# Sylphy0052/Othello_Reinforcement_learning_test

Hardware: AMD Instinct MI355X
Metric: self-play games/sec (8x8, 50 MCTS sims/move) (higher is better)
Workload: dtype f16x3 (fp16 hi/lo operand split on MFMA, fp32 accumulate; fp32-equivalent)

## Files before the change

othello_reinforcement_learning_test_amd/csrc/net_wino.hip:

```cpp
#include <math.h>
#include <stdlib.h>
#include <string.h>

#include <type_traits>
#include <vector>

#include "net.h"
#include "net_heads.h"
#include "net_epilogue.h"

namespace oth {

using half8 = _Float16 __attribute__((ext_vector_type(8)));
using half4 = _Float16 __attribute__((ext_vector_type(4)));
using f32x4 = float __attribute__((ext_vector_type(4)));

constexpr int kWTile = 512;
constexpr int kWVBytes = 2 * 32 * 4 * kWTile;
constexpr int kWZeroOff = kWVBytes;
constexpr int kWLds = kWVBytes + 4 * kWTile;
constexpr float kWClamp = 30000.0f;

struct WinoWeights {
    int blocks = 0;
    uint4* d_w = nullptr;
    uint4* d_stem = nullptr;
    float* d_bias = nullptr;
    float* d_inv = nullptr;
    float* d_pfc_wt = nullptr;
    float* d_vfc1_wt = nullptr;
};

struct WinoArgs {
    const uint4* w;
    const uint4* stem;
    const float* bias;
    const float* inv;
    int n_res_layers;
    HeadParams heads;
    const float* pfc_wt;
    const float* vfc1_wt;
    int* sat;
    float act_scale;
    unsigned long long* dbg;
};

#ifdef OTH_STAMPS
__device__ __forceinline__ unsigned long long w_clk() {
    unsigned long long t;
    __builtin_amdgcn_sched_barrier(0);
    asm volatile("s_memtime %0\n\ts_waitcnt lgkmcnt(0)" : "=s"(t)::"memory");
    __builtin_amdgcn_sched_barrier(0);
    return t;
}
__device__ __forceinline__ unsigned long long w_realclk() {
    unsigned long long t;
    __builtin_amdgcn_sched_barrier(0);
    asm volatile("s_memrealtime %0\n\ts_waitcnt lgkmcnt(0)" : "=s"(t)::"memory");
    __builtin_amdgcn_sched_barrier(0);
    return t;
}
#define OTH_WSTAMP(i) { const unsigned long long t1_ = w_clk(); ph_[i] += t1_ - t0_; t0_ = t1_; }
#else
#define OTH_WSTAMP(i)
#endif

__device__ __forceinline__ f32x4 wmfma(half8 a, half8 b, f32x4 c) {
    asm volatile("v_mfma_f32_16x16x32_f16 %0, %1, %2, %0" : "+v"(c) : "v"(a), "v"(b));
    return c;
}
__device__ __forceinline__ f32x4 wmfma0(half8 a, half8 b) {
    f32x4 c;
    asm volatile("v_mfma_f32_16x16x32_f16 %0, %1, %2, 0" : "=v"(c) : "v"(a), "v"(b));
    return c;
}
__device__ __forceinline__ void wbarrier() {
    asm volatile("s_waitcnt lgkmcnt(0)" ::: "memory");
    __builtin_amdgcn_s_barrier();
    asm volatile("" ::: "memory");
}
__device__ __forceinline__ float quad_prev(float v) {
    return __builtin_bit_cast(float, __builtin_amdgcn_mov_dpp(__builtin_bit_cast(int, v), 0x90, 0xf, 0xf, true));
}
__device__ __forceinline__ float quad_next(float v) {
    return __builtin_bit_cast(float, __builtin_amdgcn_mov_dpp(__builtin_bit_cast(int, v), 0xF9, 0xf, 0xf, true));
}

#define OTH_WSB __builtin_amdgcn_sched_barrier(0)
constexpr int kHeadRow = 129;

__device__ __forceinline__ void heads_block2(const HeadParams& hp, const float* __restrict__ pfc_wt,
                                             const float* __restrict__ vfc1_wt, const float* act, float* scratch,
                                             bool live1, float* __restrict__ logp, float* __restrict__ vout,
                                             unsigned long long* hst = nullptr) {
    const int t = threadIdx.x;
#ifdef OTH_STAMPS
    unsigned long long h0_ = w_clk();
#define OTH_HST(i) { const unsigned long long h1_ = w_clk(); if (hst) hst[i] = h1_ - h0_; h0_ = h1_; }
#else
#define OTH_HST(i)
#endif
    float* w3 = scratch;
    float* feat = scratch + 384;
    float* h1 = scratch + 768;
    float* lgp = scratch + 1280;
    if (t < 384) {
        const int i = t / 3, k = t % 3;
        w3[t] = k < 2 ? hp.pconv_w[i * 2 + k] : hp.vconv_w[i];
    }
    __syncthreads();
    if (t < 384) {
        const int p = t / 192, rem = t % 192, k = rem >> 6, cell = rem & 63;
        const float* a = act + (size_t)(p * 64 + cell) * kHeadRow;
        float p0 = 0.f, p1 = 0.f;
#pragma unroll 16
        for (int i = 0; i < 128; i += 2) {
            p0 = fmaf(a[i], w3[i * 3 + k], p0);
            p1 = fmaf(a[i + 1], w3[(i + 1) * 3 + k], p1);
        }
        float acc = p0 + p1;
        acc += k < 2 ? hp.pconv_b[k] : hp.vconv_b[0];
        feat[p * 192 + k * 64 + cell] = acc > 0.f ? acc : 0.f;
    }
    __syncthreads();
    OTH_HST(0)
    if (t < 256) {
        float a0 = hp.vfc1_b[t], a1 = a0;
#pragma unroll
        for (int i = 0; i < 64; ++i) {
            const float w = vfc1_wt[i * 256 + t];
            a0 = fmaf(w, feat[128 + i], a0);
            a1 = fmaf(w, feat[192 + 128 + i], a1);
        }
        h1[t] = a0 > 0.f ? a0 : 0.f;
        h1[256 + t] = a1 > 0.f ? a1 : 0.f;
    } else if (t < 256 + 130) {
        const int u = t - 256, o = u % 65, part = u / 65;
        float s0 = part == 0 ? hp.pfc_b[o] : 0.f, s1 = s0;
#pragma unroll
        for (int i = 0; i < 64; ++i) {
            const float w = pfc_wt[(part * 64 + i) * 65 + o];
            s0 = fmaf(w, feat[part * 64 + i], s0);
            s1 = fmaf(w, feat[192 + part * 64 + i], s1);
        }
        lgp[part * 72 + o] = s0;
        lgp[(2 + part) * 72 + o] = s1;
    }
    OTH_HST(1)
    __syncthreads();
    if ((t & 255) < 64) {
        const int p = t >> 8, l = t & 63;
        const float* gp = lgp + p * 2 * 72;
        const float gl = gp[l] + gp[72 + l];
        const float g64 = gp[64] + gp[72 + 64];
        float m = fmaxf(gl, l == 0 ? g64 : -INFINITY);
        m = bfly_max_f32(m);
        float s = expf(gl - m) + (l == 0 ? expf(g64 - m) : 0.f);
        s = bfly_sum_f32(s);
        const float lse = logf(s);
        float acc = 0.f;
        for (int i = l; i < 256; i += 64) acc = fmaf(hp.vfc2_w[i], h1[p * 256 + i], acc);
        acc = bfly_sum_f32(acc);
        if (p == 0 || live1) {
            logp[p * 65 + l] = gl - m - lse;
            if (l == 0) {
                logp[p * 65 + 64] = g64 - m - lse;
                vout[p] = tanhf(acc + hp.vfc2_b[0]);
            }
        }
    }
}

template <int TP>
__global__ __launch_bounds__(512, 2) void k_trunk_w(WinoArgs a, const uint64_t* __restrict__ sb,
                                                    const uint64_t* __restrict__ ob, const uint64_t* __restrict__ lgl,
                                                    int64_t n, const int32_t* __restrict__ n_valid,
                                                    float* __restrict__ logp, float* __restrict__ vout) {
    extern __shared__ __attribute__((aligned(16))) char lds[];
#ifdef OTH_STAMPS
    const unsigned long long tentry_ = w_clk();
#endif
    int64_t nv = n;
    if (n_valid) {
        const int64_t k = *n_valid;
        nv = k < n ? k : n;
    }
    constexpr int NT = 2 * TP;
    const int64_t pos0 = (int64_t)blockIdx.x * TP;
    if (pos0 >= nv) return;
    const int tid = threadIdx.x, lane = tid & 63, wave = tid >> 6;
    const int g4 = lane >> 4, c = lane & 15;
    const int row4 = c >> 2, j = c & 3;

    if (tid < TP * 64) {
        const int p = tid >> 6, cell = tid & 63, y = cell >> 3, x = cell & 7;
        const bool live = pos0 + p < nv;
        const uint64_t b0 = live ? sb[pos0 + p] : 0, b1 = live ? ob[pos0 + p] : 0, b2 = live ? lgl[pos0 + p] : 0;
        const _Float16 one = (x & 1) ? (_Float16)(-a.act_scale) : (_Float16)a.act_scale;
        _Float16 vals[32];
#pragma unroll
        for (int i = 0; i < 32; ++i) vals[i] = (_Float16)0.0f;
#pragma unroll
        for (int tap = 0; tap < 9; ++tap) {
            const int yy = y + tap / 3 - 1, xx = x + tap % 3 - 1;
            const bool ok = yy >= 0 && yy < 8 && xx >= 0 && xx < 8;
            const int s = ok ? yy * 8 + xx : 0;
            vals[tap * 3 + 0] = (ok && ((b0 >> s) & 1ULL)) ? one : (_Float16)0.0f;
            vals[tap * 3 + 1] = (ok && ((b1 >> s) & 1ULL)) ? one : (_Float16)0.0f;
            vals[tap * 3 + 2] = (ok && ((b2 >> s) & 1ULL)) ? one : (_Float16)0.0f;
        }
        half8* dst = (half8*)(lds + tid * 64);
#pragma unroll
        for (int q = 0; q < 4; ++q) {
            half8 t;
#pragma unroll
            for (int i = 0; i < 8; ++i) t[i] = vals[q * 8 + i];
            dst[q] = t;
        }
    }
    if (tid < 128) ((uint4*)(lds + kWZeroOff))[tid] = make_uint4(0, 0, 0, 0);
    __syncthreads();

    f32x4 acc[4][NT];
    f32x4 res[NT][2];
#pragma unroll
    for (int xi = 0; xi < 4; ++xi)
#pragma unroll
        for (int nt = 0; nt < NT; ++nt) {
            acc[xi][nt] = f32x4{0.f, 0.f, 0.f, 0.f};
            OTH_PIN_ACC(acc[xi][nt]);
        }
    OTH_PIN_ACC_END();
#pragma unroll
    for (int nt = 0; nt < NT; ++nt) res[nt][0] = res[nt][1] = f32x4{0.f, 0.f, 0.f, 0.f};

    {
        const uint4* wp = a.stem + (size_t)wave * 2 * 64 + lane;
        const half8 wh = __builtin_bit_cast(half8, wp[0]), wlo = __builtin_bit_cast(half8, wp[64]);
#pragma unroll
        for (int nt = 0; nt < NT; ++nt)
#pragma unroll
            for (int e = 0; e < 2; ++e) {
                const int cell = (nt >> 1) * 64 + ((nt & 1) * 4 + row4) * 8 + 2 * j + e;
                const half8 xh = *(const half8*)(lds + cell * 64 + g4 * 16);
                acc[3 * e][nt] = wmfma(wlo, xh, acc[3 * e][nt]);
                acc[3 * e][nt] = wmfma(wh, xh, acc[3 * e][nt]);
            }
    }

    const int ch0 = wave * 16 + 4 * g4;
    const uint32_t wchunk = (uint32_t)(2 * wave + (g4 >> 1));
    uint32_t wr_off[NT];
#pragma unroll
    for (int nt = 0; nt < NT; ++nt) {
        const uint32_t tl = (uint32_t)((nt & 1) * 16 + c);
        wr_off[nt] = ((uint32_t)(nt >> 1) * 32 + tl) * (4 * kWTile) + ((wchunk ^ (tl & 15)) << 4) + 8u * (uint32_t)(g4 & 1);
    }
    uint32_t rd_base[NT][3];
    uint32_t rd_key[3];
#pragma unroll
    for (int d = 0; d < 3; ++d) {
        rd_key[d] = ((uint32_t)((c + 4 * (d - 1)) & 15) << 4) ^ ((uint32_t)g4 << 4);
#pragma unroll
        for (int nt = 0; nt < NT; ++nt) {
            const int y = (nt & 1) * 4 + row4 + (d - 1);
            const int ts = (nt & 1) * 16 + c + 4 * (d - 1);
            rd_base[nt][d] = (y >= 0 && y < 8) ? (uint32_t)((nt >> 1) * 32 + ts) * (4 * kWTile) : (uint32_t)kWZeroOff;
        }
    }
    const float mask_l = j == 0 ? 0.f : 1.f, mask_r = j == 3 ? 0.f : 1.f;
    const f32x2 mask_l2 = {mask_l, mask_l}, mask_r2 = {mask_r, mask_r};

    const int n_layers = 1 + a.n_res_layers;
    uint32_t sat_bits = 0;
    constexpr int RING = TP == 1 ? 4 : 2;
    static_assert(12 % RING == 0, "the ring index must be a compile-time function of the group");
    uint4 wq[RING][8];
#ifdef OTH_STAMPS
    unsigned long long ph_[4] = {0, 0, 0, 0}, t0_ = w_clk(), tstart_ = t0_;
    const unsigned long long rstart_ = w_realclk();
#endif
    float4 b4 = *(const float4*)(a.bias + ch0), b4n = b4;
    float inv = a.inv[0], invn = inv;
    for (int layer = 0; layer < n_layers; ++layer) {
        const bool last = layer == n_layers - 1;
        if (layer > 0) {
            b4 = b4n;
            inv = invn;
        }
        const f32x2 inv2 = {inv, inv};
        const uint4* wl = a.w + (size_t)layer * (12 * 8 * 8 * 64) + (size_t)wave * (8 * 64) + lane;
        auto epilogue = [&](auto SKIP) {
            constexpr bool add_res = decltype(SKIP)::value;
#pragma unroll
            for (int nt = 0; nt < NT; ++nt) {
                f32x2 v0[2], v1[2];
#pragma unroll
                for (int h = 0; h < 2; ++h) {
                    const f32x2 a0 = whalf(acc[0][nt], h), a1 = whalf(acc[1][nt], h), a2 = whalf(acc[2][nt], h),
                                a3 = whalf(acc[3][nt], h);
                    const f32x2 bb = h == 0 ? f32x2{b4.x, b4.y} : f32x2{b4.z, b4.w};
                    const f32x2 t0 = pk_fma(pk_add(pk_add(a0, a1), a2), inv2, bb);
                    const f32x2 t1 = pk_fma(pk_sub(pk_sub(a1, a2), a3), inv2, bb);
                    if (add_res) {
                        f32x2 r0 = whalf(res[nt][0], h), r1 = whalf(res[nt][1], h);
                        pk_add_relu_inplace(r0, t0, kWClamp);
                        pk_add_relu_inplace(r1, t1, kWClamp);
                        wsethalf(res[nt][0], h, r0);
                        wsethalf(res[nt][1], h, r1);
                        v0[h] = r0;
                        v1[h] = r1;
                    } else {
                        v0[h] = f32x2{__builtin_amdgcn_fmed3f(t0.x, 0.f, kWClamp), __builtin_amdgcn_fmed3f(t0.y, 0.f, kWClamp)};
                        v1[h] = f32x2{__builtin_amdgcn_fmed3f(t1.x, 0.f, kWClamp), __builtin_amdgcn_fmed3f(t1.y, 0.f, kWClamp)};
                    }
                }
                sat_bits = max(sat_bits, max(max(__float_as_uint(v0[0].x), __float_as_uint(v0[0].y)),
                                             max(__float_as_uint(v0[1].x), __float_as_uint(v0[1].y))));
                sat_bits = max(sat_bits, max(max(__float_as_uint(v1[0].x), __float_as_uint(v1[0].y)),
                                             max(__float_as_uint(v1[1].x), __float_as_uint(v1[1].y))));
                if (!last) {
                    f32x2 V[4][2];
#pragma unroll
                    for (int h = 0; h < 2; ++h) {
                        const f32x2 dl = {quad_prev(v1[h].x), quad_prev(v1[h].y)};
                        const f32x2 dr = {quad_next(v0[h].x), quad_next(v0[h].y)};
                        V[0][h] = pk_fma_nc(dl, mask_l2, v1[h]);
                        V[1][h] = pk_add(v0[h], v1[h]);
                        V[2][h] = pk_sub(v1[h], v0[h]);
                        V[3][h] = pk_fma_na(dr, mask_r2, v0[h]);
                    }
#pragma unroll
                    for (int xi = 0; xi < 4; ++xi) {
                        uint2 hi, lo;
                        hi.x = wpack(V[xi][0].x, V[xi][0].y);
                        hi.y = wpack(V[xi][1].x, V[xi][1].y);
                        lo.x = wresid(hi.x, V[xi][0].x, V[xi][0].y);
                        lo.y = wresid(hi.y, V[xi][1].x, V[xi][1].y);
                        char* dst = lds + wr_off[nt] + xi * kWTile;
                        *(uint2*)dst = hi;
                        *(uint2*)(dst + 256) = lo;
                    }
                }
                OTH_WSB;
            }
        };
        using T_ = std::true_type;
        using F_ = std::false_type;
        if (layer == 0 && !last) {
#pragma unroll
            for (int g = 0; g < RING - 1; ++g)
#pragma unroll
                for (int f = 0; f < 8; ++f) wq[g][f] = wl[(size_t)g * (8 * 8 * 64) + (size_t)f * 64];
        }
        OTH_WSTAMP(0)
        wbarrier();
        OTH_WSTAMP(1)
        if (layer & 1) epilogue(F_{});
        else epilogue(T_{});
        if (last) break;
        OTH_WSTAMP(2)
        wbarrier();
        OTH_WSTAMP(1)

        constexpr int GS = NT * 4;
        constexpr int QT = 12 * GS;
        auto src_of = [&](int q) -> const char* {
            const int xi = q & 3, nt = (q >> 2) % NT, grp = q / GS, kk = grp & 3, d = grp >> 2;
            return lds + rd_base[nt][d] + ((uint32_t)(kk << 6) ^ rd_key[d]) + xi * kWTile;
        };
        constexpr int PD = 2;
        half8 xh[PD + 1], xl[PD + 1];
#pragma unroll
        for (int q = 0; q < PD; ++q) {
            xh[q] = *(const half8*)src_of(q);
            xl[q] = *(const half8*)(src_of(q) + 256);
        }
        auto conv_d = [&](auto DC) {
            constexpr int D = decltype(DC)::value;
#pragma unroll
            for (int ql = 0; ql < 4 * GS; ++ql) {
                const int q = D * 4 * GS + ql;
                const int xi = q & 3, nt = (q >> 2) % NT, grp = q / GS, sl = q % (PD + 1), psl = (q + PD) % (PD + 1);
                const int step = q % GS;
                const half8 wh = __builtin_bit_cast(half8, wq[grp % RING][2 * xi]);
                const half8 wlo = __builtin_bit_cast(half8, wq[grp % RING][2 * xi + 1]);
                OTH_WSB;
                if (q < GS) acc[xi][nt] = wmfma0(wh, xl[sl]);
                else acc[xi][nt] = wmfma(wh, xl[sl], acc[xi][nt]);
                OTH_WSB;
                if (q + PD < QT) xh[psl] = *(const half8*)src_of(q + PD);
                OTH_WSB;
                acc[xi][nt] = wmfma(wh, xh[sl], acc[xi][nt]);
                OTH_WSB;
                if (q + PD < QT) xl[psl] = *(const half8*)(src_of(q + PD) + 256);
                if (grp == 10 && step == GS / 2) {
                    b4n = *(const float4*)(a.bias + (layer + 1) * 128 + ch0);
                    invn = a.inv[layer + 1];
                }
                if (step < 8)
                    wq[(grp + RING - 1) % RING][step] = wl[(size_t)(grp + RING - 1) * (8 * 8 * 64) + (size_t)step * 64];
                OTH_WSB;
                acc[xi][nt] = wmfma(wlo, xh[sl], acc[xi][nt]);
                OTH_WSB;
            }
        };
        conv_d(std::integral_constant<int, 0>{});
        conv_d(std::integral_constant<int, 1>{});
        conv_d(std::integral_constant<int, 2>{});
        OTH_WSTAMP(3)
    }
#ifdef OTH_STAMPS
    if (a.dbg && lane == 0) {
        unsigned long long* o = a.dbg + ((size_t)blockIdx.x * 8 + wave) * 8;
        for (int i = 0; i < 4; ++i) o[i] = ph_[i];
        o[4] = w_clk() - tstart_;
        o[5] = w_realclk() - rstart_;
        o[6] = rstart_;
        o[7] = tstart_ - tentry_;
    }
    const unsigned long long theads_ = w_clk();
#endif

    if (sat_bits >= __float_as_uint(kWClamp)) atomicOr(a.sat, 1);
    __syncthreads();
#pragma unroll
    for (int nt = 0; nt < NT; ++nt)
#pragma unroll
        for (int e = 0; e < 2; ++e) {
            const int cell = (nt >> 1) * 64 + ((nt & 1) * 4 + row4) * 8 + 2 * j + e;
            const float us = 1.0f / a.act_scale;
            const f32x4 v = res[nt][e];
            float* dst = (float*)lds + (size_t)cell * kHeadRow + ch0;
            dst[0] = v[0] * us;
            dst[1] = v[1] * us;
            dst[2] = v[2] * us;
            dst[3] = v[3] * us;
        }
    __syncthreads();
#ifdef OTH_STAMPS
    unsigned long long hst_[2] = {0, 0};
    const unsigned long long tpre_ = w_clk() - theads_;
    heads_block2(a.heads, a.pfc_wt, a.vfc1_wt, (const float*)lds, (float*)(lds + 128 * kHeadRow * 4 + 64), TP == 2 && pos0 + 1 < nv,
                 logp + pos0 * 65, vout + pos0, hst_);
#if OTH_STAMPS != 2
    if (a.dbg && lane == 0) {
        unsigned long long* o = a.dbg + ((size_t)blockIdx.x * 8 + wave) * 8;
        o[3] = w_clk() - theads_;
        o[0] = tpre_; o[1] = hst_[0]; o[2] = hst_[1];
    }
#endif
#else
    heads_block2(a.heads, a.pfc_wt, a.vfc1_wt, (const float*)lds, (float*)(lds + 128 * kHeadRow * 4 + 64), TP == 2 && pos0 + 1 < nv,
                 logp + pos0 * 65, vout + pos0);
#endif
}

static inline void wsplit(float v, uint16_t& hi, uint16_t& lo) {
    const _Float16 hh = (_Float16)v;
    const _Float16 ll = (_Float16)(v - (float)hh);
    memcpy(&hi, &hh, 2);
    memcpy(&lo, &ll, 2);
}

void wino_free_weights(oth_net* net) {
    if (!net->wino) return;
    WinoWeights* w = net->wino;
    if (w->d_w) (void)hipFree(w->d_w);
    if (w->d_stem) (void)hipFree(w->d_stem);
    if (w->d_bias) (void)hipFree(w->d_bias);
    if (w->d_inv) (void)hipFree(w->d_inv);
    if (w->d_pfc_wt) (void)hipFree(w->d_pfc_wt);
    if (w->d_vfc1_wt) (void)hipFree(w->d_vfc1_wt);
    delete w;
    net->wino = nullptr;
}

int wino_pack_weights(oth_net* net) {
    const HostNet& hn = net->host;
    OTH_CHECK(hn.filters == 128 && hn.board == 8, "the Winograd trunk is built for 128 filters on 8x8");
    const int L = 2 * hn.blocks;
    WinoWeights* ww = new WinoWeights();
    ww->blocks = hn.blocks;
    net->wino = ww;
    const size_t frag = 64 * 8;
    const size_t layer_halfs = (size_t)12 * 8 * 8 * frag;
    std::vector<uint16_t> w((size_t)L * layer_halfs + 5 * 8 * 8 * frag), stem((size_t)8 * 2 * frag);
    std::vector<float> bias((size_t)(L + 1) * 128), inv(L + 1);
    {
        const FoldedConv& cv = hn.stem;
        float mx = 0.f;
        for (float x : cv.w) mx = fmaxf(mx, fabsf(x));
        int e = mx > 0.f ? (int)floorf(log2f(16384.0f / mx)) : 0;
        e = e > 24 ? 24 : (e < -24 ? -24 : e);
        const float scale = ldexpf(1.0f, e);
        for (int wv = 0; wv < 8; ++wv)
            for (int l = 0; l < 64; ++l)
                for (int jj = 0; jj < 8; ++jj) {
                    const int k = 8 * (l >> 4) + jj, co = 16 * wv + (l & 15);
                    const float v = k < 27 ? cv.w[(size_t)k * cv.cout + co] * scale : 0.f;
                    uint16_t hi, lo;
                    wsplit(v, hi, lo);
                    stem[((size_t)wv * 2 + 0) * frag + (size_t)l * 8 + jj] = hi;
                    stem[((size_t)wv * 2 + 1) * frag + (size_t)l * 8 + jj] = lo;
                }
        inv[0] = 1.0f / scale;
        for (int i = 0; i < 128; ++i) bias[i] = cv.bias[i];
    }
    static const double G[4][3] = {{1, 0, 0}, {.5, .5, .5}, {.5, -.5, .5}, {0, 0, 1}};
    std::vector<double> U((size_t)3 * 4 * 128 * 128);
    for (int li = 0; li < L; ++li) {
        const FoldedConv& cv = hn.res[li];
        double mx = 0.0;
        for (int d = 0; d < 3; ++d)
            for (int xi = 0; xi < 4; ++xi)
                for (int ci = 0; ci < 128; ++ci)
                    for (int co = 0; co < 128; ++co) {
                        double u = 0.0;
                        for (int i = 0; i < 3; ++i) u += G[xi][i] * (double)cv.w[((size_t)(d * 3 + i) * 128 + ci) * 128 + co];
                        U[(((size_t)d * 4 + xi) * 128 + ci) * 128 + co] = u;
                        mx = fmax(mx, fabs(u));
                    }
        int e = mx > 0.0 ? (int)floor(log2(16384.0 / mx)) : 0;
        e = e > 24 ? 24 : (e < -24 ? -24 : e);
        const double scale = ldexp(1.0, e);
        for (int d = 0; d < 3; ++d)
            for (int kk = 0; kk < 4; ++kk)
                for (int wv = 0; wv < 8; ++wv)
                    for (int xi = 0; xi < 4; ++xi)
                        for (int l = 0; l < 64; ++l)
                            for (int jj = 0; jj < 8; ++jj) {
                                const int ci = 32 * kk + 8 * (l >> 4) + jj, co = 16 * wv + (l & 15);
                                const float v = (float)(U[(((size_t)d * 4 + xi) * 128 + ci) * 128 + co] * scale);
                                uint16_t hi, lo;
                                wsplit(v, hi, lo);
                                const size_t f0 = (size_t)li * layer_halfs + ((((size_t)(d * 4 + kk) * 8 + wv) * 4 + xi) * 2) * frag;
                                w[f0 + (size_t)l * 8 + jj] = hi;
                                w[f0 + frag + (size_t)l * 8 + jj] = lo;
                            }
        inv[li + 1] = (float)(1.0 / scale);
        for (int i = 0; i < 128; ++i) bias[(size_t)(li + 1) * 128 + i] = cv.bias[i];
    }
    std::vector<float> pt((size_t)128 * 65), vt((size_t)64 * 256);
    for (int o = 0; o < 65; ++o)
        for (int i = 0; i < 128; ++i) pt[(size_t)i * 65 + o] = hn.pfc_w[(size_t)o * 128 + i];
    for (int o = 0; o < 256; ++o)
        for (int i = 0; i < 64; ++i) vt[(size_t)i * 256 + o] = hn.vfc1_w[(size_t)o * 64 + i];
    OTH_HIP(hipMalloc(&ww->d_pfc_wt, pt.size() * 4));
    OTH_HIP(hipMalloc(&ww->d_vfc1_wt, vt.size() * 4));
    OTH_HIP(hipMemcpy(ww->d_pfc_wt, pt.data(), pt.size() * 4, hipMemcpyHostToDevice));
    OTH_HIP(hipMemcpy(ww->d_vfc1_wt, vt.data(), vt.size() * 4, hipMemcpyHostToDevice));
    OTH_HIP(hipMalloc(&ww->d_w, w.size() * 2));
    OTH_HIP(hipMalloc(&ww->d_stem, stem.size() * 2));
    OTH_HIP(hipMalloc(&ww->d_bias, bias.size() * 4));
    OTH_HIP(hipMalloc(&ww->d_inv, inv.size() * 4));
    OTH_HIP(hipMemcpy(ww->d_w, w.data(), w.size() * 2, hipMemcpyHostToDevice));
    OTH_HIP(hipMemcpy(ww->d_stem, stem.data(), stem.size() * 2, hipMemcpyHostToDevice));
    if (int rc = register_scaled_bias(net, ww->d_bias, std::move(bias))) return rc;
    OTH_HIP(hipMemcpy(ww->d_inv, inv.data(), inv.size() * 4, hipMemcpyHostToDevice));
    return OTH_OK;
}

int wino_positions_per_workgroup(int64_t n) {
    const char* tpe = getenv("OTH_WINO_TP");
    return tpe ? (atoi(tpe) == 1 ? 1 : 2) : (n <= 256 ? 1 : 2);
}

int wino_forward(oth_net* net, const uint64_t* sb, const uint64_t* ob, const uint64_t* lg, int64_t n,
                 const int32_t* n_valid, float* logp, float* v, hipStream_t stream) {
    OTH_CHECK(net->wino, "Winograd weights not packed");
    WinoArgs a;
    a.w = net->wino->d_w;
    a.stem = net->wino->d_stem;
    a.bias = net->wino->d_bias;
    a.inv = net->wino->d_inv;
    a.n_res_layers = 2 * net->wino->blocks;
    a.heads = net->heads;
    a.pfc_wt = net->wino->d_pfc_wt;
    a.vfc1_wt = net->wino->d_vfc1_wt;
    a.sat = net->d_sat;
    a.act_scale = net->act_scale;
    a.dbg = nullptr;
#ifdef OTH_STAMPS
    const unsigned dbg_grid = (unsigned)n;
    OTH_HIP(hipMalloc(&a.dbg, (size_t)dbg_grid * 8 * 8 * sizeof(unsigned long long)));
    OTH_HIP(hipMemset(a.dbg, 0, (size_t)dbg_grid * 8 * 8 * sizeof(unsigned long long)));
#endif
    static bool attr_set_dev[64] = {};
    bool& attr_set = attr_set_dev[net->device & 63];
    if (!attr_set) {
        OTH_HIP(hipFuncSetAttribute((const void*)k_trunk_w<1>, hipFuncAttributeMaxDynamicSharedMemorySize, kWLds));
        OTH_HIP(hipFuncSetAttribute((const void*)k_trunk_w<2>, hipFuncAttributeMaxDynamicSharedMemorySize, kWLds));
        attr_set = true;
    }
    const int tp = wino_positions_per_workgroup(n);
    const unsigned grid = (unsigned)((n + tp - 1) / tp);
    if (tp == 1) hipLaunchKernelGGL(k_trunk_w<1>, dim3(grid), dim3(512), kWLds, stream, a, sb, ob, lg, n, n_valid, logp, v);
    else hipLaunchKernelGGL(k_trunk_w<2>, dim3(grid), dim3(512), kWLds, stream, a, sb, ob, lg, n, n_valid, logp, v);
    OTH_HIP(hipGetLastError());
#ifdef OTH_STAMPS
    {
        OTH_HIP(hipStreamSynchronize(stream));
        std::vector<unsigned long long> h((size_t)dbg_grid * 8 * 8);
        OTH_HIP(hipMemcpy(h.data(), a.dbg, h.size() * 8, hipMemcpyDeviceToHost));
        double sm[6] = {0, 0, 0, 0, 0, 0};
        unsigned long long r0 = ~0ull, r1 = 0;
        for (size_t w = 0; w < (size_t)dbg_grid * 8; ++w) {
            for (int i = 0; i < 6; ++i) sm[i] += (double)h[w * 8 + i];
            if (!h[w * 8 + 4]) continue;
            if (h[w * 8 + 6] < r0) r0 = h[w * 8 + 6];
            if (h[w * 8 + 6] + h[w * 8 + 5] > r1) r1 = h[w * 8 + 6] + h[w * 8 + 5];
        }
        const double nw = (double)dbg_grid * 8;
        fprintf(stderr, "[wino stamps] in-kernel clock %.3f GHz; first start -> last trunk end %.3f ms\n", sm[4] / sm[5] * 0.1,
                (double)(r1 - r0) * 1e-5);
        double pro = 0;
        for (size_t w = 0; w < (size_t)dbg_grid * 8; ++w) pro += (double)h[w * 8 + 7];
#if OTH_STAMPS == 2
        fprintf(stderr, "[wino stamps] per-wave cycles: weight prefetch %.0f | barrier waits %.0f | epilogues %.0f | convolutions %.0f | layers total %.0f | prologue+stem %.0f\n",
                sm[0] / nw * 2, sm[1] / nw * 2, sm[2] / nw * 2, sm[3] / nw * 2, sm[4] / nw * 2, pro / nw * 2);
#else
        fprintf(stderr, "[wino stamps] per-wave cycles (x2: averaged over twice the workgroups): planes->LDS %.0f | heads stage 1 (1x1 convs) %.0f | FCs %.0f | heads all %.0f | layers total %.0f | prologue+stem %.0f\n",
                sm[0] / nw, sm[1] / nw, sm[2] / nw, sm[3] / nw, sm[4] / nw, pro / nw);
#endif
        (void)hipFree(a.dbg);
    }
#endif
    return OTH_OK;
}

}
```

Baseline: 622.4.

## Prefetch head weights and trunk constants early, vectorize heads in fused trunk kernel

Packs the small head constants (conv weights, biases, vfc2) into one device buffer, loaded into LDS at kernel start. Hoists the stem weights, first weight-ring loads and bias loads ahead of the im2col stage, and splits im2col across four thread groups. The FC weights for the heads are prefetched into registers before the final activation store so their latency overlaps the epilogue. Head dot products use float4 LDS reads with padded rows, and the value-head reduction moves to separate waves. This costs extra LDS and registers, which may pressure occupancy.

```diff
diff --git a/othello_reinforcement_learning_test_amd/csrc/net_wino.hip b/othello_reinforcement_learning_test_amd/csrc/net_wino.hip
--- a/othello_reinforcement_learning_test_amd/csrc/net_wino.hip
+++ b/othello_reinforcement_learning_test_amd/csrc/net_wino.hip
@@ -18,7 +18,8 @@
 constexpr int kWTile = 512;
 constexpr int kWVBytes = 2 * 32 * 4 * kWTile;
 constexpr int kWZeroOff = kWVBytes;
-constexpr int kWLds = kWVBytes + 4 * kWTile;
+constexpr int kWHeadWOff = kWVBytes + 4 * kWTile;
+constexpr int kWLds = kWHeadWOff + 1024 * 4;
 constexpr float kWClamp = 30000.0f;
 
 struct WinoWeights {
@@ -29,6 +30,7 @@
     float* d_inv = nullptr;
     float* d_pfc_wt = nullptr;
     float* d_vfc1_wt = nullptr;
+    float* d_hc = nullptr;
 };
 
 struct WinoArgs {
@@ -37,7 +39,7 @@
     const float* bias;
     const float* inv;
     int n_res_layers;
-    HeadParams heads;
+    const float* hc;
     const float* pfc_wt;
     const float* vfc1_wt;
     int* sat;
@@ -87,10 +89,35 @@
 }
 
 #define OTH_WSB __builtin_amdgcn_sched_barrier(0)
-constexpr int kHeadRow = 129;
-
-__device__ __forceinline__ void heads_block2(const HeadParams& hp, const float* __restrict__ pfc_wt,
-                                             const float* __restrict__ vfc1_wt, const float* act, float* scratch,
+constexpr int kHeadRow = 132;
+constexpr int kHeadScratchOff = 128 * kHeadRow * 4 + 64;
+
+constexpr int kHcW3 = 0;
+constexpr int kHcCb = 384;
+constexpr int kHcV2w = 388;
+constexpr int kHcV2b = 644;
+constexpr int kHcV1b = 648;
+constexpr int kHcPb = 904;
+constexpr int kHcFloats = 1024;
+static_assert(kWLds == kWHeadWOff + kHcFloats * 4, "LDS layout");
+struct HeadsPrefetch {
+    float fw[64];
+};
+__device__ __forceinline__ void heads_prefetch(const float* __restrict__ pfc_wt, const float* __restrict__ vfc1_wt,
+                                               HeadsPrefetch& pf) {
+    const int t = threadIdx.x;
+    if (t < 256) {
+#pragma unroll
+        for (int i = 0; i < 64; ++i) pf.fw[i] = vfc1_wt[i * 256 + t];
+        asm volatile("" ::: "memory");
+    } else if (t < 256 + 130) {
+        const int u = t - 256, o = u % 65, part = u / 65;
+#pragma unroll
+        for (int i = 0; i < 64; ++i) pf.fw[i] = pfc_wt[(part * 64 + i) * 65 + o];
+    }
+}
+
+__device__ __forceinline__ void heads_block2(const HeadsPrefetch& pf, const float* act, const float* hc, float* scratch,
                                              bool live1, float* __restrict__ logp, float* __restrict__ vout,
                                              unsigned long long* hst = nullptr) {
     const int t = threadIdx.x;
@@ -100,56 +127,68 @@
 #else
 #define OTH_HST(i)
 #endif
-    float* w3 = scratch;
-    float* feat = scratch + 384;
-    float* h1 = scratch + 768;
-    float* lgp = scratch + 1280;
-    if (t < 384) {
-        const int i = t / 3, k = t % 3;
-        w3[t] = k < 2 ? hp.pconv_w[i * 2 + k] : hp.vconv_w[i];
-    }
-    __syncthreads();
+    float* feat = scratch;
+    float* h1 = scratch + 384;
+    float* lgp = scratch + 896;
     if (t < 384) {
         const int p = t / 192, rem = t % 192, k = rem >> 6, cell = rem & 63;
-        const float* a = act + (size_t)(p * 64 + cell) * kHeadRow;
+        const float4* a4 = (const float4*)(act + (size_t)(p * 64 + cell) * kHeadRow);
+        const float4* w4 = (const float4*)(hc + kHcW3 + k * 128);
         float p0 = 0.f, p1 = 0.f;
-#pragma unroll 16
-        for (int i = 0; i < 128; i += 2) {
-            p0 = fmaf(a[i], w3[i * 3 + k], p0);
-            p1 = fmaf(a[i + 1], w3[(i + 1) * 3 + k], p1);
+#pragma unroll 8
+        for (int i = 0; i < 32; ++i) {
+            const float4 av = a4[i], wv = w4[i];
+            p0 = fmaf(av.x, wv.x, p0);
+            p1 = fmaf(av.y, wv.y, p1);
+            p0 = fmaf(av.z, wv.z, p0);
+            p1 = fmaf(av.w, wv.w, p1);
         }
         float acc = p0 + p1;
-        acc += k < 2 ? hp.pconv_b[k] : hp.vconv_b[0];
+        acc += hc[kHcCb + k];
         feat[p * 192 + k * 64 + cell] = acc > 0.f ? acc : 0.f;
     }
     __syncthreads();
     OTH_HST(0)
     if (t < 256) {
-        float a0 = hp.vfc1_b[t], a1 = a0;
-#pragma unroll
-        for (int i = 0; i < 64; ++i) {
-            const float w = vfc1_wt[i * 256 + t];
-            a0 = fmaf(w, feat[128 + i], a0);
-            a1 = fmaf(w, feat[192 + 128 + i], a1);
+        float a0 = hc[kHcV1b + t], a1 = a0;
+        const float4* f0 = (const float4*)(feat + 128), * f1 = (const float4*)(feat + 192 + 128);
+#pragma unroll
+        for (int i = 0; i < 64; i += 4) {
+            const float4 x0 = f0[i >> 2], x1 = f1[i >> 2];
+            a0 = fmaf(pf.fw[i], x0.x, a0);
+            a1 = fmaf(pf.fw[i], x1.x, a1);
+            a0 = fmaf(pf.fw[i + 1], x0.y, a0);
+            a1 = fmaf(pf.fw[i + 1], x1.y, a1);
+            a0 = fmaf(pf.fw[i + 2], x0.z, a0);
+            a1 = fmaf(pf.fw[i + 2], x1.z, a1);
+            a0 = fmaf(pf.fw[i + 3], x0.w, a0);
+            a1 = fmaf(pf.fw[i + 3], x1.w, a1);
         }
         h1[t] = a0 > 0.f ? a0 : 0.f;
         h1[256 + t] = a1 > 0.f ? a1 : 0.f;
     } else if (t < 256 + 130) {
         const int u = t - 256, o = u % 65, part = u / 65;
-        float s0 = part == 0 ? hp.pfc_b[o] : 0.f, s1 = s0;
-#pragma unroll
-        for (int i = 0; i < 64; ++i) {
-            const float w = pfc_wt[(part * 64 + i) * 65 + o];
-            s0 = fmaf(w, feat[part * 64 + i], s0);
-            s1 = fmaf(w, feat[192 + part * 64 + i], s1);
+        float s0 = part == 0 ? hc[kHcPb + o] : 0.f, s1 = s0;
+        const float4* f0 = (const float4*)(feat + part * 64), * f1 = (const float4*)(feat + 192 + part * 64);
+#pragma unroll
+        for (int i = 0; i < 64; i += 4) {
+            const float4 x0 = f0[i >> 2], x1 = f1[i >> 2];
+            s0 = fmaf(pf.fw[i], x0.x, s0);
+            s1 = fmaf(pf.fw[i], x1.x, s1);
+            s0 = fmaf(pf.fw[i + 1], x0.y, s0);
+            s1 = fmaf(pf.fw[i + 1], x1.y, s1);
+            s0 = fmaf(pf.fw[i + 2], x0.z, s0);
+            s1 = fmaf(pf.fw[i + 2], x1.z, s1);
+            s0 = fmaf(pf.fw[i + 3], x0.w, s0);
+            s1 = fmaf(pf.fw[i + 3], x1.w, s1);
         }
         lgp[part * 72 + o] = s0;
         lgp[(2 + part) * 72 + o] = s1;
     }
     OTH_HST(1)
     __syncthreads();
-    if ((t & 255) < 64) {
-        const int p = t >> 8, l = t & 63;
+    const int role = t >> 6, p = role & 1, l = t & 63;
+    if (role < 2) {
         const float* gp = lgp + p * 2 * 72;
         const float gl = gp[l] + gp[72 + l];
         const float g64 = gp[64] + gp[72 + 64];
@@ -158,16 +197,16 @@
         float s = expf(gl - m) + (l == 0 ? expf(g64 - m) : 0.f);
         s = bfly_sum_f32(s);
         const float lse = logf(s);
-        float acc = 0.f;
-        for (int i = l; i < 256; i += 64) acc = fmaf(hp.vfc2_w[i], h1[p * 256 + i], acc);
-        acc = bfly_sum_f32(acc);
         if (p == 0 || live1) {
             logp[p * 65 + l] = gl - m - lse;
-            if (l == 0) {
-                logp[p * 65 + 64] = g64 - m - lse;
-                vout[p] = tanhf(acc + hp.vfc2_b[0]);
-            }
-        }
+            if (l == 0) logp[p * 65 + 64] = g64 - m - lse;
+        }
+    } else if (role < 4) {
+        float acc = 0.f;
+#pragma unroll
+        for (int i = 0; i < 4; ++i) acc = fmaf(hc[kHcV2w + l + 64 * i], h1[p * 256 + l + 64 * i], acc);
+        acc = bfly_sum_f32(acc);
+        if ((p == 0 || live1) && l == 0) vout[p] = tanhf(acc + hc[kHcV2b]);
     }
 }
 
@@ -192,33 +231,57 @@
     const int g4 = lane >> 4, c = lane & 15;
     const int row4 = c >> 2, j = c & 3;
 
-    if (tid < TP * 64) {
-        const int p = tid >> 6, cell = tid & 63, y = cell >> 3, x = cell & 7;
-        const bool live = pos0 + p < nv;
-        const uint64_t b0 = live ? sb[pos0 + p] : 0, b1 = live ? ob[pos0 + p] : 0, b2 = live ? lgl[pos0 + p] : 0;
+    constexpr int ICELLS = TP * 64;
+    const int iq = tid / ICELLS, icell = tid % ICELLS;
+    const int ip = icell >> 6;
+    const bool ilive = iq < 4 && pos0 + ip < nv;
+    const uint64_t b0 = ilive ? sb[pos0 + ip] : 0, b1 = ilive ? ob[pos0 + ip] : 0, b2 = ilive ? lgl[pos0 + ip] : 0;
+    const float hc_v0 = a.hc[tid], hc_v1 = a.hc[tid + 512];
+    const uint4* stem_p = a.stem + (size_t)wave * 2 * 64 + lane;
+    const half8 stem_h = __builtin_bit_cast(half8, stem_p[0]), stem_l = __builtin_bit_cast(half8, stem_p[64]);
+    const int ch0 = wave * 16 + 4 * g4;
+    float4 b4 = *(const float4*)(a.bias + ch0), b4n = b4;
+    float inv = a.inv[0], invn = inv;
+    constexpr int RING = TP == 1 ? 4 : 2;
+    static_assert(12 % RING == 0, "the ring index must be a compile-time function of the group");
+    uint4 wq[RING][8];
+    {
+        const uint4* wl0 = a.w + (size_t)wave * (8 * 64) + lane;
+#pragma unroll
+        for (int g = 0; g < RING - 1; ++g)
+#pragma unroll
+            for (int f = 0; f < 8; ++f) wq[g][f] = wl0[(size_t)g * (8 * 8 * 64) + (size_t)f * 64];
+    }
+
+    {
+        const int cell = icell & 63, y = cell >> 3, x = cell & 7;
         const _Float16 one = (x & 1) ? (_Float16)(-a.act_scale) : (_Float16)a.act_scale;
-        _Float16 vals[32];
-#pragma unroll
-        for (int i = 0; i < 32; ++i) vals[i] = (_Float16)0.0f;
-#pragma unroll
-        for (int tap = 0; tap < 9; ++tap) {
-            const int yy = y + tap / 3 - 1, xx = x + tap % 3 - 1;
-            const bool ok = yy >= 0 && yy < 8 && xx >= 0 && xx < 8;
-            const int s = ok ? yy * 8 + xx : 0;
-            vals[tap * 3 + 0] = (ok && ((b0 >> s) & 1ULL)) ? one : (_Float16)0.0f;
-            vals[tap * 3 + 1] = (ok && ((b1 >> s) & 1ULL)) ? one : (_Float16)0.0f;
-            vals[tap * 3 + 2] = (ok && ((b2 >> s) & 1ULL)) ? one : (_Float16)0.0f;
-        }
-        half8* dst = (half8*)(lds + tid * 64);
-#pragma unroll
-        for (int q = 0; q < 4; ++q) {
+        auto im2col_chunk = [&](auto QC) {
+            constexpr int Q = decltype(QC)::value;
             half8 t;
 #pragma unroll
-            for (int i = 0; i < 8; ++i) t[i] = vals[q * 8 + i];
-            dst[q] = t;
-        }
+            for (int i = 0; i < 8; ++i) {
+                const int k = Q * 8 + i, tap = k / 3, pl = k % 3;
+                if (k < 27) {
+                    const int yy = y + tap / 3 - 1, xx = x + tap % 3 - 1;
+                    const bool ok = yy >= 0 && yy < 8 && xx >= 0 && xx < 8;
+                    const int s = ok ? yy * 8 + xx : 0;
+                    const uint64_t bb = pl == 0 ? b0 : (pl == 1 ? b1 : b2);
+                    t[i] = (ok && ((bb >> s) & 1ULL)) ? one : (_Float16)0.0f;
+                } else {
+                    t[i] = (_Float16)0.0f;
+                }
+            }
+            *(half8*)(lds + icell * 64 + Q * 16) = t;
+        };
+        if (iq == 0) im2col_chunk(std::integral_constant<int, 0>{});
+        else if (iq == 1) im2col_chunk(std::integral_constant<int, 1>{});
+        else if (iq == 2) im2col_chunk(std::integral_constant<int, 2>{});
+        else if (iq == 3) im2col_chunk(std::integral_constant<int, 3>{});
     }
     if (tid < 128) ((uint4*)(lds + kWZeroOff))[tid] = make_uint4(0, 0, 0, 0);
+    ((float*)(lds + kWHeadWOff))[tid] = hc_v0;
+    ((float*)(lds + kWHeadWOff))[tid + 512] = hc_v1;
     __syncthreads();
 
     f32x4 acc[4][NT];
@@ -235,8 +298,7 @@
     for (int nt = 0; nt < NT; ++nt) res[nt][0] = res[nt][1] = f32x4{0.f, 0.f, 0.f, 0.f};
 
     {
-        const uint4* wp = a.stem + (size_t)wave * 2 * 64 + lane;
-        const half8 wh = __builtin_bit_cast(half8, wp[0]), wlo = __builtin_bit_cast(half8, wp[64]);
+        const half8 wh = stem_h, wlo = stem_l;
 #pragma unroll
         for (int nt = 0; nt < NT; ++nt)
 #pragma unroll
@@ -248,7 +310,6 @@
             }
     }
 
-    const int ch0 = wave * 16 + 4 * g4;
     const uint32_t wchunk = (uint32_t)(2 * wave + (g4 >> 1));
     uint32_t wr_off[NT];
 #pragma unroll
@@ -273,15 +334,10 @@
 
     const int n_layers = 1 + a.n_res_layers;
     uint32_t sat_bits = 0;
-    constexpr int RING = TP == 1 ? 4 : 2;
-    static_assert(12 % RING == 0, "the ring index must be a compile-time function of the group");
-    uint4 wq[RING][8];
 #ifdef OTH_STAMPS
     unsigned long long ph_[4] = {0, 0, 0, 0}, t0_ = w_clk(), tstart_ = t0_;
     const unsigned long long rstart_ = w_realclk();
 #endif
-    float4 b4 = *(const float4*)(a.bias + ch0), b4n = b4;
-    float inv = a.inv[0], invn = inv;
     for (int layer = 0; layer < n_layers; ++layer) {
         const bool last = layer == n_layers - 1;
         if (layer > 0) {
@@ -347,12 +403,6 @@
         };
         using T_ = std::true_type;
         using F_ = std::false_type;
-        if (layer == 0 && !last) {
-#pragma unroll
-            for (int g = 0; g < RING - 1; ++g)
-#pragma unroll
-                for (int f = 0; f < 8; ++f) wq[g][f] = wl[(size_t)g * (8 * 8 * 64) + (size_t)f * 64];
-        }
         OTH_WSTAMP(0)
         wbarrier();
         OTH_WSTAMP(1)
@@ -423,7 +473,9 @@
 #endif
 
     if (sat_bits >= __float_as_uint(kWClamp)) atomicOr(a.sat, 1);
-    __syncthreads();
+    __builtin_amdgcn_s_waitcnt(0x0F70);
+    HeadsPrefetch pf;
+    heads_prefetch(a.pfc_wt, a.vfc1_wt, pf);
 #pragma unroll
     for (int nt = 0; nt < NT; ++nt)
 #pragma unroll
@@ -431,17 +483,14 @@
             const int cell = (nt >> 1) * 64 + ((nt & 1) * 4 + row4) * 8 + 2 * j + e;
             const float us = 1.0f / a.act_scale;
             const f32x4 v = res[nt][e];
-            float* dst = (float*)lds + (size_t)cell * kHeadRow + ch0;
-            dst[0] = v[0] * us;
-            dst[1] = v[1] * us;
-            dst[2] = v[2] * us;
-            dst[3] = v[3] * us;
+            *(float4*)((float*)lds + (size_t)cell * kHeadRow + ch0) = make_float4(v[0] * us, v[1] * us, v[2] * us, v[3] * us);
         }
     __syncthreads();
+    const bool live1 = TP == 2 && pos0 + 1 < nv;
 #ifdef OTH_STAMPS
     unsigned long long hst_[2] = {0, 0};
     const unsigned long long tpre_ = w_clk() - theads_;
-    heads_block2(a.heads, a.pfc_wt, a.vfc1_wt, (const float*)lds, (float*)(lds + 128 * kHeadRow * 4 + 64), TP == 2 && pos0 + 1 < nv,
+    heads_block2(pf, (const float*)lds, (const float*)(lds + kWHeadWOff), (float*)(lds + kHeadScratchOff), live1,
                  logp + pos0 * 65, vout + pos0, hst_);
 #if OTH_STAMPS != 2
     if (a.dbg && lane == 0) {
@@ -451,7 +500,7 @@
     }
 #endif
 #else
-    heads_block2(a.heads, a.pfc_wt, a.vfc1_wt, (const float*)lds, (float*)(lds + 128 * kHeadRow * 4 + 64), TP == 2 && pos0 + 1 < nv,
+    heads_block2(pf, (const float*)lds, (const float*)(lds + kWHeadWOff), (float*)(lds + kHeadScratchOff), live1,
                  logp + pos0 * 65, vout + pos0);
 #endif
 }
@@ -472,6 +521,7 @@
     if (w->d_inv) (void)hipFree(w->d_inv);
     if (w->d_pfc_wt) (void)hipFree(w->d_pfc_wt);
     if (w->d_vfc1_wt) (void)hipFree(w->d_vfc1_wt);
+    if (w->d_hc) (void)hipFree(w->d_hc);
     delete w;
     net->wino = nullptr;
 }
@@ -546,6 +596,23 @@
         for (int i = 0; i < 128; ++i) pt[(size_t)i * 65 + o] = hn.pfc_w[(size_t)o * 128 + i];
     for (int o = 0; o < 256; ++o)
         for (int i = 0; i < 64; ++i) vt[(size_t)i * 256 + o] = hn.vfc1_w[(size_t)o * 64 + i];
+    std::vector<float> hc(kHcFloats, 0.f);
+    for (int i = 0; i < 128; ++i) {
+        hc[kHcW3 + i] = hn.pconv.w[(size_t)i * 2];
+        hc[kHcW3 + 128 + i] = hn.pconv.w[(size_t)i * 2 + 1];
+        hc[kHcW3 + 256 + i] = hn.vconv.w[i];
+    }
+    hc[kHcCb] = hn.pconv.bias[0];
+    hc[kHcCb + 1] = hn.pconv.bias[1];
+    hc[kHcCb + 2] = hn.vconv.bias[0];
+    for (int i = 0; i < 256; ++i) {
+        hc[kHcV2w + i] = hn.vfc2_w[i];
+        hc[kHcV1b + i] = hn.vfc1_b[i];
+    }
+    hc[kHcV2b] = hn.vfc2_b[0];
+    for (int o = 0; o < 65; ++o) hc[kHcPb + o] = hn.pfc_b[o];
+    OTH_HIP(hipMalloc(&ww->d_hc, hc.size() * 4));
+    OTH_HIP(hipMemcpy(ww->d_hc, hc.data(), hc.size() * 4, hipMemcpyHostToDevice));
     OTH_HIP(hipMalloc(&ww->d_pfc_wt, pt.size() * 4));
     OTH_HIP(hipMalloc(&ww->d_vfc1_wt, vt.size() * 4));
     OTH_HIP(hipMemcpy(ww->d_pfc_wt, pt.data(), pt.size() * 4, hipMemcpyHostToDevice));
@@ -575,7 +642,7 @@
     a.bias = net->wino->d_bias;
     a.inv = net->wino->d_inv;
     a.n_res_layers = 2 * net->wino->blocks;
-    a.heads = net->heads;
+    a.hc = net->wino->d_hc;
     a.pfc_wt = net->wino->d_pfc_wt;
     a.vfc1_wt = net->wino->d_vfc1_wt;
     a.sat = net->d_sat;
```

Result: no change. 625.4, median of 6 (+0.5%).
